# zxhuang1698/ZeroShape

Measured on AMD Instinct MI355X. Metric: sdf_query_points_per_sec_vox128, higher is better.
Workload: dtype f16x3

## Files before the change

### zeroshape_amd/csrc/sdf_decoder_split.hip

```cpp
#include "zs_common.h"
#include <stdlib.h>
#include "sdf_layout.h"
#include "sdf_math.h"
#include "zs_split16.h"
#include "../../include/zeroshape_hip.h"

#include <math.h>
#include <stdint.h>
#include <type_traits>

namespace {

using namespace zs::lay;
using zs::dm::gelu_erf;
using zs::dm::softplus100;

typedef float f32x16 __attribute__((ext_vector_type(16)));
typedef float f32x4 __attribute__((ext_vector_type(4)));
typedef float f32x2 __attribute__((ext_vector_type(2)));
typedef unsigned u32x4 __attribute__((ext_vector_type(4)));

constexpr float S_GUARD = 64.0f;
constexpr int WAVES = 4;
constexpr int PTS_PER_WAVE = 32;
constexpr int PTS_PER_BLOCK = WAVES * PTS_PER_WAVE;
constexpr int MAX_WGS = 256;
constexpr int KB_U4 = 128;
constexpr int CK = 8;
constexpr int KPW = CK / WAVES;
constexpr int CHUNK_BYTES = CK * KB_U4 * 16;
constexpr int NBUF = 2;
constexpr int KB_TOTAL = G_TOTAL / 2;
constexpr int PRM_WINDOW = 4096;
constexpr int STAGE_FLOATS = NBUF * CHUNK_BYTES / 4;
constexpr int SLAB_TILES = NT - 1;
constexpr int SLAB_U4 = SLAB_TILES * 4 * 64;
constexpr int ZTILES_F4 = NT * 4 * 64;
constexpr int ZSLAB_F4 = 3 * ZTILES_F4;
constexpr int LDS_FLOATS = PRM_WINDOW + STAGE_FLOATS + WAVES * SLAB_U4 * 4;
static_assert(LDS_FLOATS * 4 == 160 * 1024, "the kernel owns the whole LDS of a CU");
static_assert(KB_TOTAL % CK == 0 && CK % WAVES == 0 && KPW * 2048 <= 4096, "chunking");
static_assert((RING * GROUP_FLOATS + PARAM_FLOATS) * 4 >= NBUF * CHUNK_BYTES, "prefetch stays inside the program");

constexpr int W_PP = P_PP;
constexpr int W_BLK = P_BLK0;
constexpr int W_IA = P_LNFG;
constexpr int W_IB = P_IMPL_PAIR + P_IMPL_PAIR_STRIDE;
static_assert(P_BLK_STRIDE <= PRM_WINDOW && W_IB - W_IA <= PRM_WINDOW && P_USED - W_IB <= PRM_WINDOW,
              "params windows");

#define DEV __device__ __forceinline__
#ifdef ZS_FENCE_SCHED
#define ZS_FENCE __builtin_amdgcn_sched_barrier(0)
#else
#define ZS_FENCE do { } while (0)
#endif

DEV void pin(u32x4 &a, u32x4 &b) { asm volatile("" : "+v"(a), "+v"(b) : : "memory"); }

using zs::s16::mfma3;
using zs::s16::split2;

struct PT {
    u32x4 v[4];
};
template <typename T>
DEV PT pack_tile(const T &x) {
    PT p;
#pragma unroll
    for (int j = 0; j < 2; j++)
#pragma unroll
        for (int i = 0; i < 4; i++) {
            unsigned h, l;
            split2(x[8 * j + 2 * i], x[8 * j + 2 * i + 1], h, l);
            p.v[2 * j][i] = h;
            p.v[2 * j + 1][i] = l;
        }
    return p;
}

DEV void glds_kblocks(const char *gsrc, unsigned lds_dst) {
#ifdef ZS_EXP_NO_DMA
    if (gsrc != nullptr) return;
#endif
#ifndef ZS_DMA_MOD
#define ZS_DMA_MOD ""
#endif
    asm volatile("s_mov_b32 m0, %1\n\ts_nop 0\n\tglobal_load_lds_dwordx4 %0, off" ZS_DMA_MOD
                 "\n\tglobal_load_lds_dwordx4 %0, off offset:1024" ZS_DMA_MOD
                 "\n\tglobal_load_lds_dwordx4 %0, off offset:2048" ZS_DMA_MOD
                 "\n\tglobal_load_lds_dwordx4 %0, off offset:3072" ZS_DMA_MOD
                 :
                 : "v"(gsrc), "s"(lds_dst)
                 : "memory");
}

struct AStream {
    const u32x4 *buf[NBUF];
    unsigned dst[NBUF];
    u32x4 hi, lo;
    const char *gsrc;

    DEV void init(const char *prog, u32x4 *stage, unsigned stage_addr, int wave, int lane) {
        const char *g = prog + wave * (KPW * KB_U4 * 16) + lane * 16;
        asm volatile("s_waitcnt vmcnt(0) lgkmcnt(0)\n\ts_barrier" ::: "memory");
#pragma unroll
        for (int i = 0; i < NBUF; i++) {
            buf[i] = stage + i * (CK * KB_U4) + lane;
            dst[i] = stage_addr + i * CHUNK_BYTES + wave * (KPW * KB_U4 * 16);
            glds_kblocks(g + i * CHUNK_BYTES, dst[i]);
        }
        gsrc = g + NBUF * CHUNK_BYTES;
        asm volatile("s_waitcnt vmcnt(4)\n\ts_barrier" ::: "memory");
        hi = buf[0][0];
        lo = buf[0][64];
    }
    template <int EXTRA_VM = 0>
    DEV void step(int pos, u32x4 &ahi, u32x4 &alo) {
        ahi = hi;
        alo = lo;
        if (pos == CK - 1) {
            static_assert(EXTRA_VM == 0 || EXTRA_VM == 4, "wait-count variants");
            if (EXTRA_VM == 4)
                asm volatile("s_waitcnt vmcnt(4) lgkmcnt(0)\n\ts_barrier" ::: "memory");
            else
                asm volatile("s_waitcnt vmcnt(0) lgkmcnt(0)\n\ts_barrier" ::: "memory");
            glds_kblocks(gsrc, dst[0]);
            gsrc += CHUNK_BYTES;
            const u32x4 *t = buf[0];
            const unsigned u = dst[0];
            buf[0] = buf[1];
            dst[0] = dst[1];
            buf[1] = t;
            dst[1] = u;
            hi = buf[0][0];
            lo = buf[0][64];
        } else {
#ifndef ZS_EXP_NO_AREAD
            hi = buf[0][(pos + 1) * KB_U4];
            lo = buf[0][(pos + 1) * KB_U4 + 64];
#endif
        }
    }
    DEV void drain() { asm volatile("s_waitcnt vmcnt(0) lgkmcnt(0)" ::: "memory"); }
};

struct Slab {
    u32x4 *fl;
    PT t7;
    DEV void store(int tile, const PT &p) {
        if (tile == SLAB_TILES) {
            t7 = p;
        } else {
#pragma unroll
            for (int q = 0; q < 4; q++) fl[(tile * 4 + q) * 64] = p.v[q];
        }
    }
};

DEV f32x16 zero16() {
    f32x16 v;
#pragma unroll
    for (int r = 0; r < 16; r++) v[r] = 0.f;
    return v;
}

struct NoSide {
    DEV void operator()(int, int) const {}
};
template <typename SIDE>
DEV void mfma3_gaps(f32x16 &acc, const u32x4 &ahi, const u32x4 &alo, const u32x4 &bhi, const u32x4 &blo, int kb,
                    SIDE &side) {
    using zs::s16::as_h;
    if (std::is_same<SIDE, NoSide>::value) {
        mfma3(acc, ahi, alo, bhi, blo);
        return;
    }
    acc = __builtin_amdgcn_mfma_f32_32x32x16_f16(as_h(alo), as_h(bhi), acc, 0, 0, 0);
    ZS_FENCE;
    side(kb, 0);
    ZS_FENCE;
    acc = __builtin_amdgcn_mfma_f32_32x32x16_f16(as_h(ahi), as_h(blo), acc, 0, 0, 0);
    ZS_FENCE;
    side(kb, 1);
    ZS_FENCE;
    acc = __builtin_amdgcn_mfma_f32_32x32x16_f16(as_h(ahi), as_h(bhi), acc, 0, 0, 0);
    ZS_FENCE;
    side(kb, 2);
    ZS_FENCE;
}

struct TilePacker {
    PT p;
    float prev;
    DEV void feed(int kb, float v) {
        if (kb & 1) {
            unsigned h, l;
            split2(prev, v, h, l);
            p.v[2 * (kb >> 3)][(kb & 7) >> 1] = h;
            p.v[2 * (kb >> 3) + 1][(kb & 7) >> 1] = l;
        }
        prev = v;
    }
};

struct GeluStager {
    float x, u, q, t, e, p;
    DEV void s0(float v) {
        x = v;
        u = fabsf(v) * 0.70710678118654752440f;
        q = (u * u) * -1.44269504088896340736f;
    }
    DEV void s1() { t = __builtin_amdgcn_rcpf(fmaf(0.3275911f, u, 1.0f)); }
    DEV void s2() {
        e = __builtin_amdgcn_exp2f(q);
        p = fmaf(0.75052702f, t, -1.02753365f);
    }
    DEV void s3() {
        p = fmaf(p, t, 1.00509130f);
        p = fmaf(p, t, -0.20116957f);
        p = fmaf(p, t, 0.18019173f);
        p = p * t;
        u = u * p;
    }
    DEV float s4() const { return fmaf(-u, e, fmaxf(x, 0.0f)); }
    DEV float all(float v) {
        s0(v); s1(); s2(); s3();
        return s4();
    }
    DEV void stage(int st, float v, int idx, TilePacker &pk) {
        if (st == 0) s0(v);
        else if (st == 1) s1();
        else if (st == 2) s2();
        else if (st == 3) s3();
        else if (st == 4) pk.feed(idx, s4());
    }
};
struct SoftplusStager {
    float x, t;
    DEV void s0(float v) {
        x = v;
        t = __builtin_amdgcn_exp2f(fabsf(v) * -144.26950408889634074f);
    }
    DEV void s1() { t = __builtin_amdgcn_logf(1.0f + t); }
    DEV float s2() const { return fmaf(t, 0.0069314718055994530942f, fmaxf(x, 0.0f)); }
};

DEV float kblock_gelu(f32x16 &acc, const u32x4 &ahi, const u32x4 &alo, const u32x4 &bhi, const u32x4 &blo, float x) {
    float u, q, d, t, e, m, p;
    const float c0 = 0.70710678118654752440f, c1 = 0.3275911f, c2 = -1.02753365f;
    asm volatile(
#ifndef ZS_EXP_TWO_TERM
                 "v_mfma_f32_32x32x16_f16 %[acc], %[alo], %[bh], %[acc]\n\t"
#endif
                 "v_mul_f32_e64 %[u], |%[x]|, %[c0]\n\t"
                 "v_mul_f32_e32 %[q], %[u], %[u]\n\t"
                 "v_mul_f32_e32 %[q], 0xbfb8aa3b, %[q]\n\t"
                 "v_fma_f32 %[d], %[u], %[c1], 1.0\n\t"
                 "v_mfma_f32_32x32x16_f16 %[acc], %[ahi], %[bl], %[acc]\n\t"
                 "v_rcp_f32_e32 %[t], %[d]\n\t"
                 "v_exp_f32_e32 %[e], %[q]\n\t"
                 "v_max_f32_e32 %[m], 0, %[x]\n\t"
                 "v_mfma_f32_32x32x16_f16 %[acc], %[ahi], %[bh], %[acc]\n\t"
                 "v_fmamk_f32 %[p], %[t], 0x3f40228a, %[c2]\n\t"
                 "v_fmaak_f32 %[p], %[p], %[t], 0x3f80a6d5\n\t"
                 "v_fmaak_f32 %[p], %[p], %[t], 0xbe4dff65\n\t"
                 "v_fmaak_f32 %[p], %[p], %[t], 0x3e38842e\n\t"
                 "v_mul_f32_e64 %[p], %[t], -%[p]\n\t"
                 "v_mul_f32_e32 %[p], %[u], %[p]\n\t"
                 "v_fmac_f32_e32 %[m], %[p], %[e]"
                 : [acc] "+v"(acc), [u] "=&v"(u), [q] "=&v"(q), [d] "=&v"(d), [t] "=&v"(t), [e] "=&v"(e), [m] "=&v"(m),
                   [p] "=&v"(p)
                 : [alo] "v"(alo), [ahi] "v"(ahi), [bh] "v"(bhi), [bl] "v"(blo), [x] "v"(x), [c0] "s"(c0), [c1] "s"(c1),
                   [c2] "v"(c2));
    return m;
}
DEV float kblock_softplus(f32x16 &acc, const u32x4 &ahi, const u32x4 &alo, const u32x4 &bhi, const u32x4 &blo, float x) {
    float t, m;
    const float c0 = -144.26950408889634074f;
    asm volatile(
#ifndef ZS_EXP_TWO_TERM
// ... 43 lines not shown
}
template <int KT, typename SIDE = NoSide>
DEV void gemm_areg(AStream &s, const PT *X, f32x16 &acc, SIDE side = SIDE()) {
#pragma unroll
    for (int kt = 0; kt < KT; kt++)
#pragma unroll
        for (int j = 0; j < 2; j++) {
            u32x4 ahi, alo;
            s.step((kt * 2 + j) & (CK - 1), ahi, alo);
            pin(ahi, alo);
            mfma3_breg(acc, ahi, alo, X[kt].v[2 * j], X[kt].v[2 * j + 1], kt * 2 + j, side);
        }
}
template <typename SIDE>
DEV void mfma3_cacc(f32x16 &acc, const u32x4 &ahi, const u32x4 &alo, const u32x4 &bhi, const u32x4 &blo, int kb,
                    SIDE &side) {
    asm volatile("s_nop 1\n\tv_mfma_f32_32x32x16_f16 %0, %1, %2, %0" : "+a"(acc) : "v"(alo), "v"(bhi));
    ZS_FENCE;
    side(kb, 0);
    ZS_FENCE;
    asm volatile("s_nop 1\n\tv_mfma_f32_32x32x16_f16 %0, %1, %2, %0" : "+a"(acc) : "v"(ahi), "v"(blo));
    ZS_FENCE;
    side(kb, 1);
    ZS_FENCE;
    asm volatile("s_nop 1\n\tv_mfma_f32_32x32x16_f16 %0, %1, %2, %0" : "+a"(acc) : "v"(ahi), "v"(bhi));
    ZS_FENCE;
    side(kb, 2);
    ZS_FENCE;
}
template <bool YACC = false, typename SIDE = NoSide>
DEV void gemm_one(AStream &s, const PT &X, f32x16 &acc, int pos0, int kb0 = 0, SIDE side = SIDE()) {
#pragma unroll
    for (int j = 0; j < 2; j++) {
        u32x4 ahi, alo;
        s.step((pos0 + j) & (CK - 1), ahi, alo);
        pin(ahi, alo);
        if (YACC)
            mfma3_cacc(acc, ahi, alo, X.v[2 * j], X.v[2 * j + 1], kb0 + j, side);
        else
            mfma3_gaps(acc, ahi, alo, X.v[2 * j], X.v[2 * j + 1], kb0 + j, side);
    }
}
DEV void slab_b(const Slab &sl, int kb, u32x4 &bh, u32x4 &bl) {
    if (kb >= SLAB_TILES * 2) {
        bh = sl.t7.v[(kb & 1) * 2];
        bl = sl.t7.v[(kb & 1) * 2 + 1];
    } else {
        bh = sl.fl[kb * KB_U4];
        bl = sl.fl[kb * KB_U4 + 64];
    }
}
template <typename SIDE = NoSide>
DEV void gemm_lds(AStream &s, const Slab &sl, f32x16 &acc, int pos0 = 0, SIDE side = SIDE()) {
    u32x4 bh, bl;
    slab_b(sl, 0, bh, bl);
#pragma unroll
    for (int kb = 0; kb < NT * 2; kb++) {
        u32x4 ahi, alo;
        s.step((pos0 + kb) & (CK - 1), ahi, alo);
        u32x4 nh = bh, nl = bl;
        if (kb + 1 < NT * 2) slab_b(sl, kb + 1, nh, nl);
        pin(ahi, alo);
        mfma3_gaps(acc, ahi, alo, bh, bl, kb, side);
        bh = nh;
        bl = nl;
    }
}

template <int ACT, typename FIN, typename TAIL>
DEV void gemm_lds_act(AStream &s, const Slab &sl, f32x16 &acc, const f32x16 &cur, FIN fin, TAIL tail) {
    u32x4 bh, bl;
    slab_b(sl, 0, bh, bl);
#pragma unroll
    for (int kb = 0; kb < NT * 2; kb++) {
        u32x4 ahi, alo;
        s.step(kb & (CK - 1), ahi, alo);
        u32x4 nh = bh, nl = bl;
        if (kb + 1 < NT * 2) slab_b(sl, kb + 1, nh, nl);
        const float r = ACT == 0 ? kblock_gelu(acc, ahi, alo, bh, bl, cur[kb]) : kblock_softplus(acc, ahi, alo, bh, bl, cur[kb]);
        bh = nh;
        bl = nl;
        fin(kb, r);
        tail(kb);
    }
}
template <int ACT, typename FIN, typename TAIL>
DEV void gemm_reg_act(AStream &s, const PT *X, f32x16 &acc, const f32x16 &cur, FIN fin, TAIL tail) {
#pragma unroll
    for (int kt = 0; kt < NT; kt++)
#pragma unroll
        for (int j = 0; j < 2; j++) {
            u32x4 ahi, alo;
            const int kb = kt * 2 + j;
            s.step(kb & (CK - 1), ahi, alo);
            const float r = ACT == 0 ? kblock_gelu(acc, ahi, alo, X[kt].v[2 * j], X[kt].v[2 * j + 1], cur[kb])
                                     : kblock_softplus(acc, ahi, alo, X[kt].v[2 * j], X[kt].v[2 * j + 1], cur[kb]);
            fin(kb, r);
            tail(kb);
        }
}

#ifndef ZS_SPLIT_PERMLANE
DEV float half_sum(float v) { return v + __shfl_xor(v, 32, 64); }
DEV float half_max(float v) { return fmaxf(v, __shfl_xor(v, 32, 64)); }
#else
DEV void half_pair(float v, float &lo, float &hi) {
    lo = v;
    hi = v;
    asm volatile("s_nop 4\n\tv_permlane32_swap_b32 %0, %1\n\ts_nop 4" : "+v"(lo), "+v"(hi));
}
DEV float half_sum(float v) {
    float lo, hi;
    half_pair(v, lo, hi);
    return lo + hi;
}
#ifdef ZS_SPLIT_PERMLANE_SUM_ONLY
DEV float half_max(float v) { return fmaxf(v, __shfl_xor(v, 32, 64)); }
#else
DEV float half_max(float v) {
    float lo, hi;
    half_pair(v, lo, hi);
    return fmaxf(lo, hi);
}
#endif
#endif

DEV void rp(const float *prm, int off, int tile, int hi, float *v) {
    const f32x4 *q = reinterpret_cast<const f32x4 *>(prm + off + tile * 32 + hi * 16);
#pragma unroll
    for (int i = 0; i < 4; i++) {
        const f32x4 a = q[i];
        v[4 * i + 0] = a.x; v[4 * i + 1] = a.y; v[4 * i + 2] = a.z; v[4 * i + 3] = a.w;
    }
}
DEV f32x16 rp16(const float *prm, int off, int tile, int hi) {
    float t[16];
    rp(prm, off, tile, hi, t);
    f32x16 v;
#pragma unroll
    for (int r = 0; r < 16; r++) v[r] = t[r];
    return v;
}
DEV f32x16 xyz_affine(const float *prm, int off, int tile, int hi, float x, float y, float z) {
    const f32x4 *q = reinterpret_cast<const f32x4 *>(prm + off + tile * 128 + hi * 64);
    f32x16 v;
#pragma unroll
    for (int r = 0; r < 16; r++) {
        const f32x4 w = q[r];
        v[r] = fmaf(w.z, z, fmaf(w.y, y, fmaf(w.x, x, w.w)));
    }
    return v;
}

struct XyzInit {
    const f32x4 *q;
    f32x4 w;
    f32x16 v;
    DEV void start(const float *prm, int off, int tile, int hi) {
        q = reinterpret_cast<const f32x4 *>(prm + off + tile * 128 + hi * 64);
        w = q[0];
    }
    DEV void step(int r, float x, float y, float z) {
        v[r] = fmaf(w.z, z, fmaf(w.y, y, fmaf(w.x, x, w.w)));
        if (r + 1 < 16) w = q[r + 1];
    }
};
struct RowInit {
    const f32x4 *q;
    f32x4 w;
    f32x16 v;
    DEV void start(const float *prm, int off, int tile, int hi) {
        q = reinterpret_cast<const f32x4 *>(prm + off + tile * 32 + hi * 16);
        w = q[0];
    }
    DEV void step(int r) {
        if ((r & 3) == 0) {
            v[r] = w.x; v[r + 1] = w.y; v[r + 2] = w.z; v[r + 3] = w.w;
            if (r + 4 < 16) w = q[(r >> 2) + 1];
        }
    }
};

DEV void ln_stats(const f32x16 *x, float &mean, float &rstd) {
    float s = 0.f;
#pragma unroll
    for (int kt = 0; kt < NT; kt++)
#pragma unroll
        for (int r = 0; r < 16; r++) s += x[kt][r];
    s = half_sum(s);
    mean = s * (1.0f / 256.0f);
    float v = 0.f;
#pragma unroll
    for (int kt = 0; kt < NT; kt++)
#pragma unroll
        for (int r = 0; r < 16; r++) {
            const float d = x[kt][r] - mean;
            v = fmaf(d, d, v);
        }
    v = half_sum(v);
    rstd = 1.0f / sqrtf(v * (1.0f / 256.0f) + 1e-6f);
}
DEV void layer_norm_lds(const f32x16 *x, Slab &sl, const float *prm, int g_off, int b_off, int hi) {
    float mean, rstd;
    ln_stats(x, mean, rstd);
#pragma unroll
    for (int kt = 0; kt < NT; kt++) {
        float g[16], b[16], t[16];
        rp(prm, g_off, kt, hi, g);
        rp(prm, b_off, kt, hi, b);
#pragma unroll
        for (int r = 0; r < 16; r++) t[r] = fmaf((x[kt][r] - mean) * rstd, g[r], b[r]);
        sl.store(kt, pack_tile(t));
    }
}

DEV void load_params(float *prm, const float *prog_params, int start, int count) {
    __syncthreads();
    const f32x4 *src = reinterpret_cast<const f32x4 *>(prog_params + start);
    f32x4 *dst = reinterpret_cast<f32x4 *>(prm);
    for (int i = threadIdx.x; i < count / 4; i += WAVES * 64) dst[i] = src[i];
    __syncthreads();
}

template <bool MASK>
DEV void attn_tile(AStream &s, const PT &q, f32x16 &o, float &m_run, float &z_run, float c, int hi,
                   int pos0) {
    f32x16 S = zero16();
    gemm_one(s, q, S, pos0);
    float mt = -INFINITY;
#pragma unroll
    for (int r = 0; r < 16; r++) {
        if (MASK) {
            const int rw = (r & 3) + 8 * (r >> 2) + 4 * hi;
            S[r] = rw < L - 32 * (LT - 1) ? S[r] : -INFINITY;
        }
        mt = fmaxf(mt, S[r]);
    }
    mt *= c;
    constexpr float LAZY = 8.0f;
    if (__builtin_amdgcn_ballot_w64(mt > m_run + LAZY) != 0) {
        mt = half_max(mt);
        const float m_new = fmaxf(m_run, mt);
        const float alpha = __builtin_amdgcn_exp2f(m_run - m_new);
        z_run *= alpha;
#pragma unroll
        for (int r = 0; r < 16; r++) o[r] *= alpha;
        m_run = m_new;
    }
    float zs_ = 0.f;
#pragma unroll
    for (int r = 0; r < 16; r++) {
        const float p = __builtin_amdgcn_exp2f(fmaf(S[r], c, -m_run));
        S[r] = p;
        zs_ += p;
    }
    z_run += zs_;
    gemm_one(s, pack_tile(S), o, pos0 + 2);
}

#ifdef ZS_EXP_TIMING
#define ZS_STAMP(i) do { if (dbg) dbg[i] = __builtin_amdgcn_s_memtime(); } while (0)
#else
#define ZS_STAMP(i) do { } while (0)
#endif
DEV float decode_tile(const char *prog, float *prm, u32x4 *stage, unsigned stage_addr, u32x4 *slab,
                      f32x4 *zs, float px, float py, float pz, int wave, int lane, float &guard,
                      unsigned long long *dbg) {
    const int hi = lane >> 5;
    const float *prog_params = reinterpret_cast<const float *>(prog) + REC_FLOATS;
    AStream s;
    s.init(prog, stage, stage_addr, wave, lane);
    Slab sl;
    sl.fl = slab;
    ZS_STAMP(0);

    load_params(prm, prog_params, W_PP, 1024);
    f32x16 y[NT];
#pragma unroll
    for (int kt = 0; kt < NT; kt++) y[kt] = xyz_affine(prm, 0, kt, hi, px, py, pz);

    ZS_STAMP(1);

    const float scale = 0.17677669529663688110f;

#pragma unroll 1
    for (int blk = 0; blk < BLOCKS; blk++) {
        load_params(prm, prog_params, W_BLK + blk * P_BLK_STRIDE, P_BLK_STRIDE);
        layer_norm_lds(y, sl, prm, PB_LN1G, PB_LN1B, hi);
        ZS_STAMP(2 + blk * 4);
#pragma unroll
        for (int nt = 0; nt < NT; nt++) y[nt] += rp16(prm, PB_BPROJ, nt, hi);

        auto head = [&](int hd, auto Ptag) {
            constexpr int P = decltype(Ptag)::value;
            f32x16 q = rp16(prm, PB_BQKV, hd * 3 + 0, hi);
            gemm_lds(s, sl, q, P);
            f32x16 k = rp16(prm, PB_BQKV, hd * 3 + 1, hi);
            gemm_lds(s, sl, k, P);
            f32x16 v = rp16(prm, PB_BQKV, hd * 3 + 2, hi);
            gemm_lds(s, sl, v, P);

            const float c = scale * 1.44269504088896340736f;
            float s_self = 0.f;
            float qq = 0.f;
#pragma unroll
            for (int r = 0; r < 16; r++) {
                s_self = fmaf(q[r], k[r], s_self);
                qq = fmaf(q[r], q[r], qq);
            }
            s_self = half_sum(s_self) * c;
            {
                const float km = prog_params[P_KMAX + blk * HEADS + hd] * scale;
                guard = fmaxf(guard, half_sum(qq) * (km * km));
            }
            const PT qp = pack_tile(q);

            float m_run = -INFINITY, z_run = 0.f;
            f32x16 o = zero16();
#pragma unroll 1
            for (int l2 = 0; l2 < (LT - 1) / 2; l2++) {
                attn_tile<false>(s, qp, o, m_run, z_run, c, hi, P);
                attn_tile<false>(s, qp, o, m_run, z_run, c, hi, (P + 4) & (CK - 1));
            }
            attn_tile<true>(s, qp, o, m_run, z_run, c, hi, P);
            {
                const float m_new = fmaxf(m_run, s_self);
                const float alpha = __builtin_amdgcn_exp2f(m_run - m_new);
                const float p_self = __builtin_amdgcn_exp2f(s_self - m_new);
                const float z = fmaf(half_sum(z_run), alpha, p_self);
                const float inv = 1.0f / z;
                const float a_i = alpha * inv, p_i = p_self * inv;
#pragma unroll
                for (int r = 0; r < 16; r++) o[r] = fmaf(p_i, v[r], o[r] * a_i);
            }
            const PT op = pack_tile(o);
#pragma unroll
            for (int nt = 0; nt < NT; nt++) gemm_one(s, op, y[nt], (P + 4 + 2 * nt) & (CK - 1));
        };
        static_assert((LT - 1) % 2 == 0 && (3 * NT * 2 + LT * 4 + NT * 2) % CK == 4, "head = 11.5 chunks");
#pragma unroll 1
        for (int hd = 0; hd < HEADS; hd += 2) {
            head(hd, std::integral_constant<int, 0>());
            head(hd + 1, std::integral_constant<int, 4>());
        }

        ZS_STAMP(3 + blk * 4);
        layer_norm_lds(y, sl, prm, PB_LN2G, PB_LN2B, hi);
#pragma unroll
        for (int nt = 0; nt < NT; nt++) y[nt] += rp16(prm, PB_B2, nt, hi);
        ZS_STAMP(4 + blk * 4);
        RowInit bi;
        f32x16 hid = rp16(prm, PB_B1, 0, hi);
        bi.start(prm, PB_B1, 1, hi);
        gemm_lds(s, sl, hid, 0, [&](int kb, int g) {
            if (g == 2 && (kb & 3) == 1) bi.step(kb & ~3);
        });
#pragma unroll 1
        for (int ht = 0; ht < HT - 1; ht++) {
            f32x16 nxt = bi.v;
            bi.start(prm, PB_B1, ht + 2 < HT ? ht + 2 : HT - 1, hi);
            TilePacker e;
            gemm_lds_act<0>(s, sl, nxt, hid, [&](int kb, float r) { e.feed(kb, r); },
                            [&](int kb) { if ((kb & 3) == 1) bi.step(kb & ~3); });
#pragma unroll
            for (int nt = 0; nt < NT; nt++) gemm_one(s, e.p, y[nt], (2 * nt) & (CK - 1));
            hid = nxt;
        }
        {
#pragma unroll
            for (int r = 0; r < 16; r++) hid[r] = gelu_erf(hid[r]);
            const PT hp = pack_tile(hid);
#pragma unroll
            for (int nt = 0; nt < NT; nt++) gemm_one(s, hp, y[nt], (2 * nt) & (CK - 1));
        }
        ZS_STAMP(5 + blk * 4);
    }

    load_params(prm, prog_params, W_IA, W_IB - W_IA);
    float h[NT * 16];
    {
        float mean, rstd;
        ln_stats(y, mean, rstd);
#pragma unroll
        for (int kt = 0; kt < NT; kt++) {
            float g[16], b[16];
            rp(prm, P_LNFG - W_IA, kt, hi, g);
            rp(prm, P_LNFB - W_IA, kt, hi, b);
#pragma unroll
            for (int r = 0; r < 16; r++) h[kt * 16 + r] = fmaf((y[kt][r] - mean) * rstd, g[r], b[r]);
        }
    }
    ZS_STAMP(10);
    PT hp[NT];

#pragma unroll
    for (int kt = 0; kt < NT; kt++) hp[kt] = pack_tile(h + kt * 16);
    {
        f32x16 prev;
        XyzInit ini;
        ini.v = xyz_affine(prm, P_IMPL0 - W_IA, 0, hi, px, py, pz);
#pragma unroll
        for (int nt = 0; nt <= NT; nt++) {
            TilePacker e;
            if (nt < NT) {
                f32x16 acc = ini.v;
                if (nt + 1 < NT) ini.start(prm, P_IMPL0 - W_IA, nt + 1, hi);
                if (nt > 0)
                    gemm_reg_act<1>(s, hp, acc, prev, [&](int kb, float r) { e.feed(kb, r); },
                                    [&](int kb) { if (nt + 1 < NT) ini.step(kb, px, py, pz); });
                else
                    gemm_reg<NT, 0>(s, hp, acc, [&](int kb, int g) { if (g == 2) ini.step(kb, px, py, pz); });
                if (nt > 0) sl.store(nt - 1, e.p);
                prev = acc;
            } else {
#pragma unroll
                for (int kb = 0; kb < 16; kb++) e.feed(kb, softplus100(prev[kb]));
                sl.store(nt - 1, e.p);
            }
        }
    }
    ZS_STAMP(11);
    const float rsqrt2 = 0.70710678118654752440f;
    PT fp[NT];
#pragma unroll
    for (int kt = 0; kt < NT; kt++) {
        float t[16];
#pragma unroll
        for (int r = 0; r < 16; r++) t[r] = h[kt * 16 + r] * rsqrt2;
        fp[kt] = pack_tile(t);
    }
    const float sx = px * rsqrt2, sy = py * rsqrt2, sz = pz * rsqrt2;

    ZS_STAMP(12);
    {
        f32x16 prev;
        RowInit ini;
        ini.v = rp16(prm, P_IMPL1 - W_IA, 0, hi);
#pragma unroll
        for (int nt = 0; nt <= NT; nt++) {
            TilePacker e;
            if (nt < NT) {
                f32x16 acc = ini.v;
                if (nt + 1 < NT) ini.start(prm, P_IMPL1 - W_IA, nt + 1, hi);
                if (nt > 0)
                    gemm_lds_act<1>(s, sl, acc, prev, [&](int kb, float r) { e.feed(kb, r * rsqrt2); },
                                    [&](int kb) { if (nt + 1 < NT) ini.step(kb); });
                else
                    gemm_lds(s, sl, acc, 0, [&](int kb, int g) { if (g == 2) ini.step(kb); });
                if (nt > 0) hp[nt - 1] = e.p;
                prev = acc;
            } else {
#pragma unroll
                for (int kb = 0; kb < 16; kb++) e.feed(kb, softplus100(prev[kb]) * rsqrt2);
                hp[nt - 1] = e.p;
            }
        }
    }
    ZS_STAMP(13);
    float out = 0.f;
#pragma unroll 1
    for (int i = 0; i < 3; i++) {
        if (i == 1) load_params(prm, prog_params, W_IB, P_USED - W_IB);
        const int pp = i == 0 ? P_IMPL_PAIR - W_IA : (i - 1) * P_IMPL_PAIR_STRIDE;
        {
            f32x16 prev;
            XyzInit ini;
            ini.v = xyz_affine(prm, pp, 0, hi, sx, sy, sz);
#pragma unroll
            for (int nt = 0; nt <= NT; nt++) {
                TilePacker e;
                if (nt < NT) {
                    f32x16 acc = ini.v;
                    if (nt + 1 < NT) ini.start(prm, pp, nt + 1, hi);
                    if (nt > 0)
                        gemm_reg_act<1>(s, hp, acc, prev, [&](int kb, float r) { e.feed(kb, r); }, [&](int) {});
                    else
                        gemm_reg<NT>(s, hp, acc);
                    gemm_areg<NT>(s, fp, acc, [&](int kb, int g) {
                        if (g == 2 && nt + 1 < NT) ini.step(kb, sx, sy, sz);
                    });
                    if (nt > 0) sl.store(nt - 1, e.p);
                    prev = acc;
                } else {
#pragma unroll
                    for (int kb = 0; kb < 16; kb++) e.feed(kb, softplus100(prev[kb]));
                    sl.store(nt - 1, e.p);
                }
            }
        }
        const float post = i < 2 ? rsqrt2 : 1.0f;
        {
            f32x16 prev;
            RowInit ini, w8;
            const float wsel = i == 2 ? 1.0f : 0.0f;
            ini.v = rp16(prm, pp + 1024, 0, hi);
#pragma unroll
            for (int r = 0; r < 16; r++) w8.v[r] = 0.f;
#pragma unroll
            for (int nt = 0; nt <= NT; nt++) {
                TilePacker e;
                const f32x16 w = w8.v * wsel;
                auto finish = [&](int kb, float v) {
                    const float t = v * post;
                    e.feed(kb, t);
                    out = fmaf(t, w[kb], out);
                };
                if (nt < NT) {
                    f32x16 acc = ini.v;
                    if (nt + 1 < NT) ini.start(prm, pp + 1024, nt + 1, hi);
                    w8.start(prm, P_W8 - W_IB, nt, hi);
                    auto tail = [&](int kb) {
                        if (nt + 1 < NT) ini.step(kb);
                        w8.step(kb);
                    };
                    if (nt > 0)
                        gemm_lds_act<1>(s, sl, acc, prev, [&](int kb, float r) { finish(kb, r); }, tail);
                    else
                        gemm_lds(s, sl, acc, 0, [&](int kb, int g) { if (g == 2) tail(kb); });
                    if (nt > 0) hp[nt - 1] = e.p;
                    prev = acc;
                } else {
#pragma unroll
                    for (int kb = 0; kb < 16; kb++) finish(kb, softplus100(prev[kb]));
                    hp[nt - 1] = e.p;
                }
            }
        }
    }
    ZS_STAMP(14);
// ... 326 lines not shown
```

### zeroshape_amd/csrc/sdf_layout.h

```cpp
#pragma once

namespace zs {
namespace lay {

constexpr int C = 256, NT = 8, HEADS = 8, HD = 32, L = 197, LT = 7, HID = 1024, HT = 32;
constexpr int BLOCKS = 2;
constexpr int GROUP_FLOATS = 256;
constexpr int RING = 8;

constexpr int G_QKV_HEAD = 3 * NT * 4;
constexpr int G_KV_HEAD = LT * 8;
constexpr int G_PROJ_HEAD = NT * 4;
constexpr int G_HEAD = G_QKV_HEAD + G_KV_HEAD + G_PROJ_HEAD;
constexpr int G_MLP_TILE = 64;
constexpr int G_BLOCK = HEADS * G_HEAD + HT * G_MLP_TILE;
constexpr int G_IMPL = 256 * 5 + 512 * 3;
constexpr int G_TOTAL = BLOCKS * G_BLOCK + G_IMPL;
constexpr int REC_FLOATS = (G_TOTAL + RING) * GROUP_FLOATS;
constexpr int PARAM_FLOATS = 13824;
constexpr int PROGRAM_FLOATS = REC_FLOATS + PARAM_FLOATS;

constexpr int P_PP = 0;
constexpr int P_BLK0 = 1024;
constexpr int P_BLK_STRIDE = 3328;
constexpr int PB_LN1G = 0, PB_LN1B = 256, PB_BPROJ = 512, PB_BQKV = 768, PB_LN2G = 1536,
              PB_LN2B = 1792, PB_B2 = 2048, PB_B1 = 2304;
constexpr int P_LNFG = 7680, P_LNFB = 7936;
constexpr int P_IMPL0 = 8192;
constexpr int P_IMPL1 = 9216;
constexpr int P_IMPL_PAIR = 9472;
constexpr int P_IMPL_PAIR_STRIDE = 1280;
constexpr int P_W8 = 13312, P_B8 = 13568;
constexpr int P_USED = 13584;
constexpr int P_FLAG = 13600;
constexpr int P_KMAX = 13616;
constexpr int P_PHASE_B = 8192;

constexpr int LQ_WLP = 0, LQ_BLP = 65536, LQ_POS = 65792, LQ_LN1G0 = 116224, LQ_LN1B0 = 116480,
              LQ_WQKV0 = 116736, LQ_BQKV0 = 313344, LQ_WPROJ0 = 314112, LQ_BPROJ0 = 379648,
              LQ_LN2G0 = 379904, LQ_LN2B0 = 380160, LQ_W1 = 380416, LQ_B1 = 642560,
              LQ_W2 = 643584, LQ_B2 = 905728, LQ_LN1G1 = 905984, LQ_LN1B1 = 906240,
              LQ_WKV1 = 906496, LQ_BKV1 = 1037568, LQ_TOTAL = 1038080;

constexpr int LPAD = 200;
constexpr int S_LAT = 0;
constexpr int S_X1 = S_LAT + LPAD * C;
constexpr int S_X2 = S_X1 + LPAD * C;
constexpr int S_QKV0 = S_X2 + LPAD * C;
constexpr int S_ATT = S_QKV0 + LPAD * 3 * C;
constexpr int S_HID = S_ATT + LPAD * C;
constexpr int S_KV1 = S_HID + LPAD * HID;
constexpr int SCRATCH_FLOATS = S_KV1 + LPAD * 2 * C;

}
}
```

### zeroshape_amd/program.py

```python
import numpy as np

C = 256
NT = C // 32
HEADS = 8
HD = 32
L = 197
LT = 7
HID = 1024
HT = HID // 32
BLOCKS = 2
MLP_LAYERS = 9
SKIP_IN = (2, 4, 6)
GROUP_FLOATS = 256
RING = 8

LANE = np.arange(64)
LANE_I = LANE & 31
LANE_HI = LANE >> 5


def row(r, hi):
    return (r & 3) + 8 * (r >> 2) + 4 * hi


ROW_TABLE = np.array([[row(r, hi) for r in range(16)] for hi in range(2)])


def _records_linear(W, nt, kt):
    rows = 32 * nt + LANE_I
    cols = 32 * kt + ROW_TABLE[LANE_HI][:, :].T
    return W[rows[None, :], cols]


def _interleave(recs):
    n = recs.shape[0]
    assert n % 4 == 0
    return recs.reshape(n // 4, 4, 64).transpose(0, 2, 1).reshape(-1)


def records_for_linear(W, n_out_tiles=None, k_tiles=None):
    W = np.asarray(W, np.float32)
    n_out_tiles = W.shape[0] // 32 if n_out_tiles is None else n_out_tiles
    k_tiles = W.shape[1] // 32 if k_tiles is None else k_tiles
    out = [_records_linear(W, nt, kt) for nt in range(n_out_tiles) for kt in range(k_tiles)]
    return np.concatenate(out, axis=0)


def kv_records(K_h, V_h):
    Kp = np.zeros((LT * 32, HD), np.float32)
    Vp = np.zeros((LT * 32, HD), np.float32)
    Kp[:L], Vp[:L] = K_h, V_h
    out = []
    for lt in range(LT):
        krec = Kp[(32 * lt + LANE_I)[None, :], ROW_TABLE[LANE_HI].T]
        vrec = Vp[32 * lt + ROW_TABLE[LANE_HI].T, LANE_I[None, :]]
        out += [krec, vrec]
    return np.concatenate(out, axis=0)


G_QKV_HEAD = 3 * NT * 4
G_KV_HEAD = LT * 8
G_PROJ_HEAD = NT * 4
G_HEAD = G_QKV_HEAD + G_KV_HEAD + G_PROJ_HEAD
G_MLP_TILE = NT * 4 + NT * 4
G_BLOCK = HEADS * G_HEAD + HT * G_MLP_TILE
G_IMPL_PLAIN = NT * NT * 4
G_IMPL_SKIP = 2 * G_IMPL_PLAIN
G_IMPL = G_IMPL_PLAIN * 5 + G_IMPL_SKIP * 3
G_TOTAL = BLOCKS * G_BLOCK + G_IMPL
REC_FLOATS = (G_TOTAL + RING) * GROUP_FLOATS
PARAM_FLOATS = 13824
PROGRAM_FLOATS = REC_FLOATS + PARAM_FLOATS
PROGRAM_BYTES = PROGRAM_FLOATS * 4


def kv_group_offset(blk, head):
    return blk * G_BLOCK + head * G_HEAD + G_QKV_HEAD


def pack_records(sd, kv=None):
    out = []
    for blk in range(BLOCKS):
        p = "blocks_attn.%d." % blk
        Wqkv = np.asarray(sd[p + "attn.qkv.weight"], np.float32)
        Wproj = np.asarray(sd[p + "attn.proj.weight"], np.float32)
        W1 = np.asarray(sd[p + "mlp.fc1.weight"], np.float32)
        W2 = np.asarray(sd[p + "mlp.fc2.weight"], np.float32)
        for h in range(HEADS):
            for part in range(3):
                Wt = Wqkv[part * C + h * HD: part * C + (h + 1) * HD]
                out.append(records_for_linear(Wt))
            if kv is not None:
                out.append(kv_records(*kv[(blk, h)]))
            else:
                out.append(np.zeros((G_KV_HEAD * 4, 64), np.float32))
            out.append(records_for_linear(Wproj[:, h * HD:(h + 1) * HD]))
        for ht in range(HT):
            out.append(records_for_linear(W1[ht * 32:(ht + 1) * 32]))
            out.append(records_for_linear(W2[:, ht * 32:(ht + 1) * 32]))
    Wl = [np.asarray(sd["impl_mlp.layers.%d.weight" % l], np.float32) for l in range(MLP_LAYERS)]
    out.append(records_for_linear(Wl[0][:, 3:]))
    for l in SKIP_IN:
        out.append(records_for_linear(Wl[l][:, C + 3:]))
    for l in range(1, MLP_LAYERS - 1):
        if l in SKIP_IN:
            out.append(records_for_linear(Wl[l][:, :C]))
        else:
            out.append(records_for_linear(Wl[l]))
    recs = np.concatenate(out, axis=0)
    assert recs.shape == (G_TOTAL * 4, 64), recs.shape
    flat = _interleave(recs)
    out = np.concatenate([flat, np.zeros(RING * GROUP_FLOATS, np.float32)])
    assert out.size == REC_FLOATS
    return out


def rowparam(v):
    v = np.asarray(v, np.float32)
    T = v.shape[0] // 32
    idx = (32 * np.arange(T))[:, None, None] + ROW_TABLE[None, :, :]
    return v[idx].reshape(-1)


def rowparam4(cols):
    stacked = np.stack([rowparam(c).reshape(-1) for c in cols], axis=-1)
    return stacked.reshape(-1)


class ParamLayout(object):

    def __init__(self):
        o = 0

        def take(n):
            nonlocal o
            s = o
            o += n
            return s
        self.PP = take(C * 4)
        self.blk = []
        for _ in range(BLOCKS):
            d = {}
            d["ln1_g"] = take(C)
            d["ln1_b"] = take(C)
            d["bproj"] = take(C)
            d["bqkv"] = take(HEADS * 3 * 32)
            d["ln2_g"] = take(C)
            d["ln2_b"] = take(C)
            d["b2"] = take(C)
            d["b1"] = take(HID)
            self.blk.append(d)
        self.lnf_g = take(C)
        self.lnf_b = take(C)
        self.impl = []
        for l in range(MLP_LAYERS - 1):
            if l == 0 or l in SKIP_IN:
                self.impl.append(take(C * 4))
            else:
                self.impl.append(take(C))
        self.w8 = take(C)
        self.b8 = take(16)
        self.total = o


PARAMS = ParamLayout()
assert PARAMS.total <= PARAM_FLOATS
P_FLAG = 13600
P_KMAX = 13616
assert PARAMS.total <= P_FLAG and P_FLAG + 4 <= P_KMAX and P_KMAX + BLOCKS * HEADS <= PARAM_FLOATS
BLOCK_PARAM_FLOATS = 3 * C + HEADS * 96 + 3 * C + HID


def pack_params(sd):
    g = lambda k: np.asarray(sd[k], np.float32)
    out = np.zeros(PARAM_FLOATS, np.float32)

    def put(off, arr):
        out[off:off + arr.size] = arr
    Wp = g("point_proj.proj.weight")
    put(PARAMS.PP, rowparam4([Wp[:, 0], Wp[:, 1], Wp[:, 2], g("point_proj.proj.bias")]))
    for blk in range(BLOCKS):
        p, d = "blocks_attn.%d." % blk, PARAMS.blk[blk]
        put(d["ln1_g"], rowparam(g(p + "norm1.weight")))
        put(d["ln1_b"], rowparam(g(p + "norm1.bias")))
        put(d["bproj"], rowparam(g(p + "attn.proj.bias")))
        bq = g(p + "attn.qkv.bias")
        parts = []
        for h in range(HEADS):
            for part in range(3):
                parts.append(rowparam(bq[part * C + h * HD: part * C + (h + 1) * HD]))
        put(d["bqkv"], np.concatenate(parts))
        put(d["ln2_g"], rowparam(g(p + "norm2.weight")))
        put(d["ln2_b"], rowparam(g(p + "norm2.bias")))
        put(d["b2"], rowparam(g(p + "mlp.fc2.bias")))
        put(d["b1"], rowparam(g(p + "mlp.fc1.bias")))
    put(PARAMS.lnf_g, rowparam(g("norm.weight")))
    put(PARAMS.lnf_b, rowparam(g("norm.bias")))
    for l in range(MLP_LAYERS - 1):
        W, b = g("impl_mlp.layers.%d.weight" % l), g("impl_mlp.layers.%d.bias" % l)
        if l == 0:
            put(PARAMS.impl[l], rowparam4([W[:, 0], W[:, 1], W[:, 2], b]))
        elif l in SKIP_IN:
            put(PARAMS.impl[l], rowparam4([W[:, C], W[:, C + 1], W[:, C + 2], b]))
        else:
            put(PARAMS.impl[l], rowparam(b))
    put(PARAMS.w8, rowparam(g("impl_mlp.layers.8.weight")[0]))
    out[PARAMS.b8] = g("impl_mlp.layers.8.bias")[0]
    return out


def pack_program(sd, kv=None):
    out = np.concatenate([pack_records(sd, kv), pack_params(sd)])
    assert out.size == PROGRAM_FLOATS
    return out


class LatentLayout(object):
    def __init__(self, latent_dim=C):
        o = 0

        def take(n):
            nonlocal o
            s = o
            o += n
            return s
        self.latent_dim = latent_dim
        self.Wlp = take(latent_dim * C)
        self.blp = take(C)
        self.pos = take(L * C)
        self.ln1g0 = take(C)
        self.ln1b0 = take(C)
        self.Wqkv0 = take(C * 3 * C)
        self.bqkv0 = take(3 * C)
        self.Wproj0 = take(C * C)
        self.bproj0 = take(C)
        self.ln2g0 = take(C)
        self.ln2b0 = take(C)
        self.W1 = take(C * HID)
        self.b1 = take(HID)
        self.W2 = take(HID * C)
        self.b2 = take(C)
        self.ln1g1 = take(C)
        self.ln1b1 = take(C)
        self.Wkv1 = take(C * 2 * C)
        self.bkv1 = take(2 * C)
        self.total = o


LATENT = LatentLayout()


def pack_latent_params(sd):
    g = lambda k: np.asarray(sd[k], np.float32)
    assert g("latent_proj.weight").shape == (C, LATENT.latent_dim)
    out = np.zeros(LATENT.total, np.float32)

    def put(off, arr):
        arr = np.ascontiguousarray(arr, np.float32).reshape(-1)
        out[off:off + arr.size] = arr
    put(LATENT.Wlp, g("latent_proj.weight").T)
    put(LATENT.blp, g("latent_proj.bias"))
    put(LATENT.pos, g("pos_embed").reshape(L, C))
    b0, b1 = "blocks_attn.0.", "blocks_attn.1."
    put(LATENT.ln1g0, g(b0 + "norm1.weight"))
    put(LATENT.ln1b0, g(b0 + "norm1.bias"))
    put(LATENT.Wqkv0, g(b0 + "attn.qkv.weight").T)
    put(LATENT.bqkv0, g(b0 + "attn.qkv.bias"))
    put(LATENT.Wproj0, g(b0 + "attn.proj.weight").T)
    put(LATENT.bproj0, g(b0 + "attn.proj.bias"))
    put(LATENT.ln2g0, g(b0 + "norm2.weight"))
    put(LATENT.ln2b0, g(b0 + "norm2.bias"))
    put(LATENT.W1, g(b0 + "mlp.fc1.weight").T)
    put(LATENT.b1, g(b0 + "mlp.fc1.bias"))
    put(LATENT.W2, g(b0 + "mlp.fc2.weight").T)
    put(LATENT.b2, g(b0 + "mlp.fc2.bias"))
    put(LATENT.ln1g1, g(b1 + "norm1.weight"))
    put(LATENT.ln1b1, g(b1 + "norm1.bias"))
    put(LATENT.Wkv1, g(b1 + "attn.qkv.weight")[C:].T)
    put(LATENT.bkv1, g(b1 + "attn.qkv.bias")[C:])
    return out


LPAD = 200
SCRATCH_FLOATS = LPAD * (3 * C + 3 * C + C + HID + 2 * C)


KB_TOTAL = G_TOTAL // 2
KB_WORDS = 512


def split_source_kblocks(n=None):
    n = REC_FLOATS // GROUP_FLOATS // 2 if n is None else n
    src = np.arange(n)
    kb_block, kb_att = G_BLOCK // 2, HEADS * G_HEAD // 2
    order = list(range(16))
    for t in range(HT - 1):
        order += [(t + 1) * 32 + r for r in range(16)] + [t * 32 + 16 + r for r in range(16)]
    order += [(HT - 1) * 32 + 16 + r for r in range(16)]
    assert sorted(order) == list(range(HT * 32))
    for blk in range(BLOCKS):
        base = blk * kb_block + kb_att
        src[base:base + HT * 32] = base + np.array(order)
    b0, kl = BLOCKS * kb_block, NT * NT * 2
    impl = list(range(kl)) + [4 * kl + i for i in range(kl)]
    for pair in range(3):
        for nt in range(NT):
            impl += [(5 + 2 * pair) * kl + nt * 2 * NT + w for w in range(2 * NT)]
            impl += [(1 + pair) * kl + nt * 2 * NT + w for w in range(2 * NT)]
        impl += [(6 + 2 * pair) * kl + i for i in range(kl)]
    assert sorted(impl) == list(range(G_IMPL // 2))
    src[b0:b0 + G_IMPL // 2] = b0 + np.array(impl)
    return src


def f16_round(x):
    x = np.ascontiguousarray(x, np.float32)
    with np.errstate(over="ignore"):
        h = x.astype(np.float16)
    return h.view(np.uint16), h.astype(np.float32)


def f16_rtz(x):
    x = np.ascontiguousarray(x, np.float32)
    with np.errstate(over="ignore"):
        h = x.astype(np.float16)
    away = np.abs(h.astype(np.float32)) > np.abs(x)
    h = np.where(away, np.nextafter(h, np.float16(0)), h).astype(np.float16)
    return h.view(np.uint16), h.astype(np.float32)


def split_program(prog):
    prog = np.ascontiguousarray(prog, np.float32)
    rec = prog[:REC_FLOATS].reshape(-1, 2, 64, 4)
    rec = rec[split_source_kblocks(rec.shape[0])]
    vals = rec.transpose(0, 2, 1, 3).reshape(-1, 64, 8)
    hi16, hif = f16_round(vals)
    with np.errstate(invalid="ignore"):
        lo16, _ = f16_round(vals - hif)
    out = np.stack([hi16, lo16], axis=1)
    words = np.ascontiguousarray(out).reshape(-1).view(np.uint32)
    params = prog[REC_FLOATS:].copy()
    params[P_KMAX:P_KMAX + BLOCKS * HEADS] = latent_k_bounds(prog).reshape(-1)
    bad = not (np.all(np.isfinite(prog)) and float(np.abs(prog).max()) <= F16_MAX)
    params[P_FLAG:P_FLAG + 1].view(np.uint32)[0] = 1 if bad else 0
    return np.concatenate([words, params.view(np.uint32)])


S_GUARD = 64.0
W_MAX = 16.0
F16_MAX = 65504.0


def split_envelope(sd):
    vals = [np.asarray(v, np.float32) for k, v in sd.items() if k != "pos_embed"]
    wmax = max(float(np.max(np.abs(v))) if np.all(np.isfinite(v)) else float("inf") for v in vals)
    return wmax <= W_MAX, dict(max_abs_weight=wmax)


def latent_k_bounds(prog):
    prog = np.ascontiguousarray(prog, np.float32)
    out = np.zeros((BLOCKS, HEADS), np.float32)
    for blk in range(BLOCKS):
        for h in range(HEADS):
            o = kv_group_offset(blk, h) * GROUP_FLOATS
            g = prog[o:o + G_KV_HEAD * GROUP_FLOATS].reshape(LT, 8, 64, 4)[:, :4]
            rec = g.transpose(0, 1, 3, 2).reshape(LT, 16, 64)
            sq = (rec.astype(np.float64) ** 2).sum(1)
            row = sq[:, :32] + sq[:, 32:]
            out[blk, h] = np.sqrt(row.max())
    return out
```

Measured before the change: 75.09 million.

## Fold block-0 LayerNorm and QKV projection into a per-point affine table

Block 0's input is the point projection of xyz, so LayerNorm followed by the QKV GEMM reduces to an affine function of xyz scaled by rstd. The host now precomputes a 4-column table plus a bias for each QKV row. The kernel evaluates q/k/v per head with a few FMAs instead of streaming and running the QKV MFMA GEMMs. The weight stream skips the block-0 QKV kblocks, which cuts global traffic and matrix work. The cost is a larger parameter region and a separately loaded block-0 parameter window, and the folded table carries its own rounding error.

```diff
diff --git a/zeroshape_amd/csrc/sdf_decoder_split.hip b/zeroshape_amd/csrc/sdf_decoder_split.hip
--- a/zeroshape_amd/csrc/sdf_decoder_split.hip
+++ b/zeroshape_amd/csrc/sdf_decoder_split.hip
@@ -31,6 +31,9 @@
 constexpr int CHUNK_BYTES = CK * KB_U4 * 16;
 constexpr int NBUF = 2;
 constexpr int KB_TOTAL = G_TOTAL / 2;
+constexpr int B0_SKIP_KB = G_QKV_HEAD / 2;
+constexpr int B0_HEAD_KB = G_HEAD / 2 - B0_SKIP_KB;
+constexpr int KB_FETCHED = KB_TOTAL - HEADS * B0_SKIP_KB;
 constexpr int PRM_WINDOW = 4096;
 constexpr int STAGE_FLOATS = NBUF * CHUNK_BYTES / 4;
 constexpr int SLAB_TILES = NT - 1;
@@ -40,14 +43,17 @@
 constexpr int LDS_FLOATS = PRM_WINDOW + STAGE_FLOATS + WAVES * SLAB_U4 * 4;
 static_assert(LDS_FLOATS * 4 == 160 * 1024, "the kernel owns the whole LDS of a CU");
 static_assert(KB_TOTAL % CK == 0 && CK % WAVES == 0 && KPW * 2048 <= 4096, "chunking");
+static_assert(B0_SKIP_KB % KPW == 0 && B0_HEAD_KB % KPW == 0 && (HEADS * B0_HEAD_KB) % CK == 0 && KB_FETCHED % CK == 0,
+              "block-0 skip schedule");
 static_assert((RING * GROUP_FLOATS + PARAM_FLOATS) * 4 >= NBUF * CHUNK_BYTES, "prefetch stays inside the program");
 
 constexpr int W_PP = P_PP;
 constexpr int W_BLK = P_BLK0;
 constexpr int W_IA = P_LNFG;
 constexpr int W_IB = P_IMPL_PAIR + P_IMPL_PAIR_STRIDE;
-static_assert(P_BLK_STRIDE <= PRM_WINDOW && W_IB - W_IA <= PRM_WINDOW && P_USED - W_IB <= PRM_WINDOW,
-              "params windows");
+constexpr int W_B0 = P_B0;
+static_assert(P_BLK_STRIDE <= PRM_WINDOW && W_IB - W_IA <= PRM_WINDOW && P_USED - W_IB <= PRM_WINDOW &&
+              B0_FLOATS == PRM_WINDOW && P_B0 + B0_FLOATS <= PARAM_FLOATS, "params windows");
 
 #define DEV __device__ __forceinline__
 #ifdef ZS_FENCE_SCHED
@@ -100,9 +106,12 @@
     unsigned dst[NBUF];
     u32x4 hi, lo;
     const char *gsrc;
+    int vpos;
+    int vhead;
 
     DEV void init(const char *prog, u32x4 *stage, unsigned stage_addr, int wave, int lane) {
-        const char *g = prog + wave * (KPW * KB_U4 * 16) + lane * 16;
+        const char *g = prog + (B0_SKIP_KB * KB_U4 * 16) + wave * (KPW * KB_U4 * 16) + lane * 16;
+        static_assert(NBUF * CK <= B0_HEAD_KB, "the chunks staged by init() lie in head 0");
         asm volatile("s_waitcnt vmcnt(0) lgkmcnt(0)\n\ts_barrier" ::: "memory");
 #pragma unroll
         for (int i = 0; i < NBUF; i++) {
@@ -111,6 +120,8 @@
             glds_kblocks(g + i * CHUNK_BYTES, dst[i]);
         }
         gsrc = g + NBUF * CHUNK_BYTES;
+        vpos = wave * KPW + NBUF * CK;
+        vhead = B0_HEAD_KB;
         asm volatile("s_waitcnt vmcnt(4)\n\ts_barrier" ::: "memory");
         hi = buf[0][0];
         lo = buf[0][64];
@@ -126,7 +137,10 @@
             else
                 asm volatile("s_waitcnt vmcnt(0) lgkmcnt(0)\n\ts_barrier" ::: "memory");
             glds_kblocks(gsrc, dst[0]);
-            gsrc += CHUNK_BYTES;
+            vpos += CK;
+            const bool jump = vpos >= vhead;
+            gsrc += jump ? CHUNK_BYTES + B0_SKIP_KB * KB_U4 * 16 : CHUNK_BYTES;
+            vhead = !jump ? vhead : vhead + B0_HEAD_KB < HEADS * B0_HEAD_KB ? vhead + B0_HEAD_KB : 0x7fffffff;
             const u32x4 *t = buf[0];
             const unsigned u = dst[0];
             buf[0] = buf[1];
@@ -476,6 +490,15 @@
     return v;
 }
 
+DEV f32x16 b0_tile(const float *prm, int tile, int hi, float x, float y, float z, float rstd) {
+    asm volatile("" ::: "memory");
+    const f32x16 t = xyz_affine(prm, B0_TAB, tile, hi, x, y, z);
+    f32x16 v = rp16(prm, B0_QKV0, tile, hi);
+#pragma unroll
+    for (int r = 0; r < 16; r++) v[r] = fmaf(rstd, t[r], v[r]);
+    return v;
+}
+
 struct XyzInit {
     const f32x4 *q;
     f32x4 w;
@@ -538,10 +561,10 @@
     }
 }
 
-DEV void load_params(float *prm, const float *prog_params, int start, int count) {
+DEV void load_params(float *prm, const float *prog_params, int start, int count, int at = 0) {
     __syncthreads();
     const f32x4 *src = reinterpret_cast<const f32x4 *>(prog_params + start);
-    f32x4 *dst = reinterpret_cast<f32x4 *>(prm);
+    f32x4 *dst = reinterpret_cast<f32x4 *>(prm + at);
     for (int i = threadIdx.x; i < count / 4; i += WAVES * 64) dst[i] = src[i];
     __syncthreads();
 }
@@ -607,22 +630,36 @@
 
     const float scale = 0.17677669529663688110f;
 
-#pragma unroll 1
-    for (int blk = 0; blk < BLOCKS; blk++) {
-        load_params(prm, prog_params, W_BLK + blk * P_BLK_STRIDE, P_BLK_STRIDE);
-        layer_norm_lds(y, sl, prm, PB_LN1G, PB_LN1B, hi);
+    auto block = [&](auto Btag) {
+        constexpr int blk = decltype(Btag)::value;
+        float rstd0 = 0.f;
+        if constexpr (blk == 0) {
+            load_params(prm, prog_params, W_B0, B0_FLOATS);
+            float mean;
+            ln_stats(y, mean, rstd0);
+        } else {
+            load_params(prm, prog_params, W_BLK + blk * P_BLK_STRIDE, P_BLK_STRIDE);
+            layer_norm_lds(y, sl, prm, PB_LN1G, PB_LN1B, hi);
+        }
         ZS_STAMP(2 + blk * 4);
 #pragma unroll
-        for (int nt = 0; nt < NT; nt++) y[nt] += rp16(prm, PB_BPROJ, nt, hi);
+        for (int nt = 0; nt < NT; nt++) y[nt] += rp16(prm, blk == 0 ? B0_BPROJ : PB_BPROJ, nt, hi);
 
         auto head = [&](int hd, auto Ptag) {
             constexpr int P = decltype(Ptag)::value;
-            f32x16 q = rp16(prm, PB_BQKV, hd * 3 + 0, hi);
-            gemm_lds(s, sl, q, P);
-            f32x16 k = rp16(prm, PB_BQKV, hd * 3 + 1, hi);
-            gemm_lds(s, sl, k, P);
-            f32x16 v = rp16(prm, PB_BQKV, hd * 3 + 2, hi);
-            gemm_lds(s, sl, v, P);
+            f32x16 q, k, v;
+            if constexpr (blk == 0) {
+                q = b0_tile(prm, hd * 3 + 0, hi, px, py, pz, rstd0);
+                k = b0_tile(prm, hd * 3 + 1, hi, px, py, pz, rstd0);
+                v = b0_tile(prm, hd * 3 + 2, hi, px, py, pz, rstd0);
+            } else {
+                q = rp16(prm, PB_BQKV, hd * 3 + 0, hi);
+                gemm_lds(s, sl, q, P);
+                k = rp16(prm, PB_BQKV, hd * 3 + 1, hi);
+                gemm_lds(s, sl, k, P);
+                v = rp16(prm, PB_BQKV, hd * 3 + 2, hi);
+                gemm_lds(s, sl, v, P);
+            }
 
             const float c = scale * 1.44269504088896340736f;
             float s_self = 0.f;
@@ -661,12 +698,15 @@
 #pragma unroll
             for (int nt = 0; nt < NT; nt++) gemm_one(s, op, y[nt], (P + 4 + 2 * nt) & (CK - 1));
         };
-        static_assert((LT - 1) % 2 == 0 && (3 * NT * 2 + LT * 4 + NT * 2) % CK == 4, "head = 11.5 chunks");
+        static_assert((LT - 1) % 2 == 0 && (3 * NT * 2 + LT * 4 + NT * 2) % CK == 4 && B0_HEAD_KB % CK == 4,
+                      "head = 11.5 chunks, 5.5 in block 0");
 #pragma unroll 1
         for (int hd = 0; hd < HEADS; hd += 2) {
             head(hd, std::integral_constant<int, 0>());
             head(hd + 1, std::integral_constant<int, 4>());
         }
+        if constexpr (blk == 0)
+            load_params(prm, prog_params, W_BLK + PB_LN2G, P_BLK_STRIDE - PB_LN2G, PB_LN2G);
 
         ZS_STAMP(3 + blk * 4);
         layer_norm_lds(y, sl, prm, PB_LN2G, PB_LN2B, hi);
@@ -698,7 +738,10 @@
             for (int nt = 0; nt < NT; nt++) gemm_one(s, hp, y[nt], (2 * nt) & (CK - 1));
         }
         ZS_STAMP(5 + blk * 4);
-    }
+    };
+    static_assert(BLOCKS == 2, "block 0, block 1");
+    block(std::integral_constant<int, 0>());
+    block(std::integral_constant<int, 1>());
 
     load_params(prm, prog_params, W_IA, W_IB - W_IA);
     float h[NT * 16];
diff --git a/zeroshape_amd/csrc/sdf_layout.h b/zeroshape_amd/csrc/sdf_layout.h
--- a/zeroshape_amd/csrc/sdf_layout.h
+++ b/zeroshape_amd/csrc/sdf_layout.h
@@ -17,7 +17,7 @@
 constexpr int G_IMPL = 256 * 5 + 512 * 3;
 constexpr int G_TOTAL = BLOCKS * G_BLOCK + G_IMPL;
 constexpr int REC_FLOATS = (G_TOTAL + RING) * GROUP_FLOATS;
-constexpr int PARAM_FLOATS = 13824;
+constexpr int PARAM_FLOATS = 17920;
 constexpr int PROGRAM_FLOATS = REC_FLOATS + PARAM_FLOATS;
 
 constexpr int P_PP = 0;
@@ -34,6 +34,11 @@
 constexpr int P_USED = 13584;
 constexpr int P_FLAG = 13600;
 constexpr int P_KMAX = 13616;
+constexpr int P_B0 = 13824;
+constexpr int B0_BPROJ = 0;
+constexpr int B0_QKV0 = 256;
+constexpr int B0_TAB = 1024;
+constexpr int B0_FLOATS = 4096;
 constexpr int P_PHASE_B = 8192;
 
 constexpr int LQ_WLP = 0, LQ_BLP = 65536, LQ_POS = 65792, LQ_LN1G0 = 116224, LQ_LN1B0 = 116480,
diff --git a/zeroshape_amd/program.py b/zeroshape_amd/program.py
--- a/zeroshape_amd/program.py
+++ b/zeroshape_amd/program.py
@@ -69,7 +69,7 @@
 G_IMPL = G_IMPL_PLAIN * 5 + G_IMPL_SKIP * 3
 G_TOTAL = BLOCKS * G_BLOCK + G_IMPL
 REC_FLOATS = (G_TOTAL + RING) * GROUP_FLOATS
-PARAM_FLOATS = 13824
+PARAM_FLOATS = 17920
 PROGRAM_FLOATS = REC_FLOATS + PARAM_FLOATS
 PROGRAM_BYTES = PROGRAM_FLOATS * 4
 
@@ -167,8 +167,25 @@
 assert PARAMS.total <= PARAM_FLOATS
 P_FLAG = 13600
 P_KMAX = 13616
+P_B0 = 13824
+B0_BPROJ = 0
+B0_QKV0 = 256
+B0_TAB = 1024
+B0_FLOATS = 4096
+assert P_KMAX + BLOCKS * HEADS <= P_B0 and P_B0 + B0_FLOATS == PARAM_FLOATS
 assert PARAMS.total <= P_FLAG and P_FLAG + 4 <= P_KMAX and P_KMAX + BLOCKS * HEADS <= PARAM_FLOATS
 BLOCK_PARAM_FLOATS = 3 * C + HEADS * 96 + 3 * C + HID
+
+
+def block0_tables(sd):
+    g = lambda k: np.asarray(sd[k], np.float32).astype(np.float64)
+    Wpp, bpp = g("point_proj.proj.weight"), g("point_proj.proj.bias")
+    ln_g, ln_b = g("blocks_attn.0.norm1.weight"), g("blocks_attn.0.norm1.bias")
+    W, b = g("blocks_attn.0.attn.qkv.weight"), g("blocks_attn.0.attn.qkv.bias")
+    Cc = Wpp - Wpp.mean(axis=0, keepdims=True)
+    c0 = bpp - bpp.mean()
+    A = np.concatenate([(W * ln_g[None, :]) @ Cc, ((W * ln_g[None, :]) @ c0)[:, None]], axis=1)
+    return A, W @ ln_b + b
 
 
 def pack_params(sd):
@@ -206,6 +223,11 @@
             put(PARAMS.impl[l], rowparam(b))
     put(PARAMS.w8, rowparam(g("impl_mlp.layers.8.weight")[0]))
     out[PARAMS.b8] = g("impl_mlp.layers.8.bias")[0]
+    put(P_B0 + B0_BPROJ, rowparam(g("blocks_attn.0.attn.proj.bias")))
+    A, q0 = block0_tables(sd)
+    order = np.concatenate([part * C + h * HD + np.arange(HD) for h in range(HEADS) for part in range(3)])
+    put(P_B0 + B0_QKV0, rowparam(q0[order].astype(np.float32)))
+    put(P_B0 + B0_TAB, rowparam4([A[order, j].astype(np.float32) for j in range(4)]))
     return out
 
 
@@ -287,6 +309,26 @@
 
 KB_TOTAL = G_TOTAL // 2
 KB_WORDS = 512
+KB_HEAD = G_HEAD // 2
+KB_QKV_HEAD = G_QKV_HEAD // 2
+KB_FETCHED = KB_TOTAL - HEADS * KB_QKV_HEAD
+CK, STAGE_WAVES = 8, 4
+
+
+def split_fetch_schedule(wave, chunks=None):
+    chunks = KB_FETCHED // CK if chunks is None else chunks
+    kb_head = KB_HEAD - KB_QKV_HEAD
+    src = KB_QKV_HEAD + 2 * wave
+    vpos, bound = 2 * wave, kb_head
+    out = []
+    for _ in range(chunks):
+        out.append((src, src + 1))
+        vpos += CK
+        src += CK
+        if vpos >= bound:
+            src += KB_QKV_HEAD
+            bound = bound + kb_head if bound + kb_head < HEADS * kb_head else 1 << 30
+    return np.array(out)
 
 
 def split_source_kblocks(n=None):
```

Measured after the change: 26.69 million. 0.356x the previous value.
